# X-PLUG/Youku-mPLUG

Measured on NVIDIA H100. Metric: video-text samples/sec (pretrain 1.3B, 8f x 224^2), higher is better.
Workload: dtype bf16

## Files before the change

include/ymp.h:

```cpp
#ifndef YMP_H_
#define YMP_H_

#include <stddef.h>
#include <stdint.h>

#ifdef __cplusplus
extern "C" {
#endif

#define YMP_OK 0
#define YMP_EINVAL (-1)
#define YMP_ECUDA (-2)
#define YMP_ENOSUP (-3)

const char* ymp_last_error(void);
int ymp_abi_version(void);
uint64_t ymp_launch_count(void);
int ymp_set_pdl(int on);

typedef struct ymp_dropout_spec {
  const uint64_t* rng;
  uint32_t site;
  float p;
} ymp_dropout_spec;
#define YMP_DROP_SITE_EMBED 0u
#define YMP_DROP_SITE_ATTN(layer) (4u * (layer) + 1u)
#define YMP_DROP_SITE_BDA_ATTN(layer) (4u * (layer) + 2u)
#define YMP_DROP_SITE_BDA_MLP(layer) (4u * (layer) + 3u)

#define YMP_ACT_NONE 0
#define YMP_ACT_GELU_ERF 1
#define YMP_ACT_GELU_TANH 2

#define YMP_DT_BF16 0
#define YMP_DT_F32 1

typedef struct ymp_gemm_args {
  const void* A;
  const void* B;
  void* D;
  int32_t M, N, K;
  int32_t lda, ldb, ldd;
  int32_t a_mn_major, b_mn_major;
  const void* bias;
  const void* residual;
  int32_t ldr;
  int32_t act;
  void* aux_out;
  const void* aux_in;
  int32_t out_dtype;
  int32_t accumulate;
  int32_t split_k;
  float alpha;
  int32_t tile_n;
  int32_t res_row_mod;
  int32_t d_row_block;
  int32_t d_row_stride;
  int32_t residual_dtype;
  ymp_dropout_spec drop;
  int32_t im2col_P, im2col_B, im2col_C, im2col_T, im2col_H, im2col_W;
} ymp_gemm_args;

int ymp_gemm(const ymp_gemm_args* a, void* stream);

typedef struct ymp_gemm_skinny_args {
  const void* x;
  const void* w;
  const void* bias;
  const void* residual;
  void* y;
  int32_t M, N, K, ldx, ldw, ldr, ldy;
  int32_t act, residual_dtype, out_dtype;
  void* y2;
  const int64_t* y2_off_dev;
  int64_t ldy2, y2_off_stride;
  const void* ln_gamma;
  const void* ln_beta;
  void* ln_out;
  uint32_t* ln_counter;
  int32_t ld_ln;
  float ln_eps;
} ymp_gemm_skinny_args;
int ymp_gemm_skinny(const ymp_gemm_skinny_args* a, void* stream);
int ymp_gemm_skinny_wide(const ymp_gemm_skinny_args* a, void* stream);

typedef struct ymp_layernorm_args {
  const void* x;
  const void* gamma;
  const void* beta;
  void* y;
  float* mean;
  float* rstd;
  const int32_t* in_rows;
  int32_t rows, D, ldx, ldy;
  float eps;
  int32_t x_dtype;
  int32_t y_dtype;
} ymp_layernorm_args;
int ymp_layernorm_fwd(const ymp_layernorm_args* a, void* stream);

typedef struct ymp_layernorm_bwd_args {
  const void* dy;
  const void* x;
  const void* gamma;
  const float* mean;
  const float* rstd;
  const void* add;
  void* dx;
  float* dgamma;
  float* dbeta;
  const int32_t* in_rows;
  int32_t rows, D, ldx, lddy, ldadd;
  int32_t x_dtype;
  void* dx_drop;
  ymp_dropout_spec drop;
} ymp_layernorm_bwd_args;
// ... 140 lines not shown
```

youku-mplug_b200/csrc/gemm_wgmma.cu:

```cuda
#include <cuda.h>

#include "common.h"
#include "philox.cuh"
#include "ptx.cuh"
#include "wgmma.cuh"

namespace ymp {

constexpr int BM = 128;
constexpr int BK = 64;
constexpr int WGMMA_K = 16;
constexpr int GEMM_THREADS = 3 * 128;
constexpr int A_STAGE_BYTES = BM * BK * 2;

struct GemmKParams {
  void* D;
  const __nv_bfloat16* bias;
  const void* residual;
  __nv_bfloat16* aux_out;
  const __nv_bfloat16* aux_in;
  int M, N, K;
  int ldd, ldr;
  int a_mn, b_mn;
  int act, out_f32, accumulate, split_k;
  int kb_per_split;
  int res_row_mod;
  int d_row_block, d_row_stride;
  int res_f32;
  int n_fast;
  float alpha;
  int im2col_T, im2col_N, im2col_Wp;
  DropSpec drop;
  int has_drop;
};

template <int BN>
struct GemmCfg {
  static constexpr int NSTAGE = (BN == 256) ? 4 : 6;
  static constexpr int B_STAGE_BYTES = BN * BK * 2;
  static constexpr int STAGE_BYTES = A_STAGE_BYTES + B_STAGE_BYTES;
  static constexpr int STG_LD = BN + 4;
  static_assert(BM * STG_LD * 4 <= NSTAGE * STAGE_BYTES, "epilogue staging reuses the operand ring");
  static constexpr int SMEM_BYTES = NSTAGE * STAGE_BYTES + 256 + 1024;
};

template <int BN>
struct EpiCfg {
  static constexpr int TPR = BN / 8;
  static constexpr int RPP = 256 / TPR;
  static constexpr int GROUP = 4;
  static_assert(BM % (RPP * GROUP) == 0, "row groups tile BM");
};

__device__ __forceinline__ uint2 ld_bf16x4(const __nv_bfloat16* p) { return __ldg(reinterpret_cast<const uint2*>(p)); }
__device__ __forceinline__ void st_bf16x4(__nv_bfloat16* p, const float* f) {
  *reinterpret_cast<uint2*>(p) = make_uint2(pack_bf16(f[0], f[1]), pack_bf16(f[2], f[3]));
}

constexpr int EPI_ANY = -1;
enum { EPI_AUX_NONE = 0, EPI_AUX_MUL = 1, EPI_AUX_GELU_ERF = 2, EPI_AUX_GELU_TANH = 3 };
enum { EPI_OUT_BF16 = 0, EPI_OUT_F32 = 1, EPI_OUT_ATOMIC = 2 };
constexpr int epi_kind(int aux, int res_f32, int out) { return aux * 16 + res_f32 * 4 + out; }
template <int KIND>
struct EpiFlags {
  bool aux_in, aux_out, residual, res_f32, out_f32, accumulate;
  int act;
  __device__ __forceinline__ explicit EpiFlags(const GemmKParams& p) {
    if constexpr (KIND == EPI_ANY) {
      aux_in = p.aux_in != nullptr; aux_out = p.aux_out != nullptr; act = p.act;
      residual = p.residual != nullptr; res_f32 = p.res_f32 != 0;
      out_f32 = p.out_f32 != 0; accumulate = p.accumulate != 0;
    } else {
      constexpr int aux = KIND / 16, out = KIND % 4;
      aux_in = aux == EPI_AUX_MUL; aux_out = aux >= EPI_AUX_GELU_ERF;
      act = aux == EPI_AUX_GELU_ERF ? YMP_ACT_GELU_ERF : aux == EPI_AUX_GELU_TANH ? YMP_ACT_GELU_TANH : YMP_ACT_NONE;
      residual = res_f32 = (KIND / 4) % 4 != 0;
      out_f32 = out != EPI_OUT_BF16; accumulate = out == EPI_OUT_ATOMIC;
    }
  }
};
__device__ __forceinline__ int epi_kind_of(const GemmKParams& p) {
  const int aux = p.aux_in ? EPI_AUX_MUL
                  : (p.act == YMP_ACT_NONE && !p.aux_out) ? EPI_AUX_NONE
                  : (p.act == YMP_ACT_GELU_ERF && p.aux_out) ? EPI_AUX_GELU_ERF
                  : (p.act == YMP_ACT_GELU_TANH && p.aux_out) ? EPI_AUX_GELU_TANH : -1;
  if (aux < 0 || p.has_drop || (p.residual && !p.res_f32)) return EPI_ANY;
  return epi_kind(aux, p.residual ? 1 : 0, !p.out_f32 ? EPI_OUT_BF16 : p.accumulate ? EPI_OUT_ATOMIC : EPI_OUT_F32);
}

struct EpiIn {
  uint32_t res[8];
  uint32_t aux[4];
};
template <int KIND>
__device__ __forceinline__ void epilogue_fetch(const GemmKParams& p, int row, const int (&col)[2], bool full, EpiIn& in) {
  const EpiFlags<KIND> f(p);
  if (row >= p.M || !full) return;
  if (f.aux_in) {
#pragma unroll
    for (int q = 0; q < 2; ++q) {
      const uint2 a = ld_bf16x4(p.aux_in + (size_t)row * p.ldd + col[q]);
      in.aux[2 * q] = a.x; in.aux[2 * q + 1] = a.y;
// ... 76 lines not shown
        for (int i = 0; i < 8; ++i) v[i] += __uint_as_float(in.res[i]);
      } else {
#pragma unroll
        for (int i = 0; i < 4; ++i) { v[2 * i] += bf16_lo(in.res[i]); v[2 * i + 1] += bf16_hi(in.res[i]); }
      }
    }
#pragma unroll
    for (int q = 0; q < 2; ++q) {
      if (!f.out_f32) {
        st_bf16x4(reinterpret_cast<__nv_bfloat16*>(p.D) + doff[q], v + 4 * q);
      } else if (!f.accumulate) {
        *reinterpret_cast<float4*>(reinterpret_cast<float*>(p.D) + doff[q]) = make_float4(v[4 * q], v[4 * q + 1], v[4 * q + 2], v[4 * q + 3]);
      } else {
        asm volatile("red.global.add.v4.f32 [%0], {%1, %2, %3, %4};" ::"l"(reinterpret_cast<float*>(p.D) + doff[q]),
                     "f"(v[4 * q]), "f"(v[4 * q + 1]), "f"(v[4 * q + 2]), "f"(v[4 * q + 3])
                     : "memory");
      }
    }
  } else {
#pragma unroll
    for (int i = 0; i < 8; ++i) {
      const int c = col[i >> 2] + (i & 3);
      if (c < p.N) {
        float x = v[i];
        if (p.bias) x += __bfloat162float(p.bias[c]);
        const size_t off = (size_t)row * p.ldd + c, doff = (size_t)drow * p.ldd + c;
        if (f.aux_in) {
          x *= __bfloat162float(p.aux_in[off]);
        } else if (f.act == YMP_ACT_GELU_ERF) {
          float d; x = gelu_erf_both(x, d);
          if (f.aux_out) p.aux_out[off] = __float2bfloat16(d);
        } else if (f.act == YMP_ACT_GELU_TANH) {
          float d; x = gelu_tanh_both(x, d);
          if (f.aux_out) p.aux_out[off] = __float2bfloat16(d);
        } else if (f.aux_out) {
          p.aux_out[off] = __float2bfloat16(x);
        }
        if constexpr (DROP) {
          const uint4 w = drop_words(ds, (uint32_t)row, (uint32_t)c >> 2);
          const uint32_t wc = (c & 3) == 0 ? w.x : (c & 3) == 1 ? w.y : (c & 3) == 2 ? w.z : w.w;
          x = wc >= ds.thresh ? x * ds.scale : 0.f;
        }
        if (f.residual)
          x += f.res_f32 ? reinterpret_cast<const float*>(p.residual)[(size_t)rrow * p.ldr + c]
                         : __bfloat162float(reinterpret_cast<const __nv_bfloat16*>(p.residual)[(size_t)rrow * p.ldr + c]);
        if (!f.out_f32) reinterpret_cast<__nv_bfloat16*>(p.D)[doff] = __float2bfloat16(x);
        else if (!f.accumulate) reinterpret_cast<float*>(p.D)[doff] = x;
        else atomicAdd(reinterpret_cast<float*>(p.D) + doff, x);
      }
    }
  }
}

constexpr int IM2COL_SUB_BYTES = BM * 32;
__device__ __forceinline__ void load_a_im2col(uint8_t* sa, const CUtensorMap* tma, uint64_t* bar, int m0, int kb,
                                              const GemmKParams& p) {
  const int T = p.im2col_T, c = kb >> 2, y0 = (kb & 3) * 4;
  const int pt = m0 / T;
  for (int i = 0; i < BM / T; ++i) {
    const int g = pt + i, b = g / p.im2col_N, n = g - b * p.im2col_N;
    const int ny = n / p.im2col_Wp, nx = n - ny * p.im2col_Wp;
#pragma unroll
    for (int ks = 0; ks < 4; ++ks) {
      uint8_t* dst = sa + ks * IM2COL_SUB_BYTES + i * T * 32;
      tma_load_5d(dst, tma, bar, nx * 16, ny * 16 + y0 + ks, 0, c, b);
    }
  }
}
__device__ __forceinline__ void named_sync(int id, int n) { asm volatile("bar.sync %0, %1;" ::"r"(id), "r"(n) : "memory"); }

template <int BN, int KIND>
__device__ __forceinline__ void epilogue_rows(const GemmKParams& p, const float* stg, int m_blk, int n_blk) {
  using Cfg = GemmCfg<BN>;
  using Epi = EpiCfg<BN>;
  DropState ds;
  if (KIND == EPI_ANY && p.has_drop) ds = drop_state(p.drop);
  const int et = threadIdx.x - 128, tj = et % Epi::TPR, tr = et / Epi::TPR;
  const int col[2] = {n_blk * BN + 4 * tj, n_blk * BN + BN / 2 + 4 * tj};
  const bool full = col[1] + 4 <= p.N;
  uint32_t bias[4];
  if (p.bias && full) {
#pragma unroll
    for (int q = 0; q < 2; ++q) {
      const uint2 b = ld_bf16x4(p.bias + col[q]);
      bias[2 * q] = b.x; bias[2 * q + 1] = b.y;
    }
  }
#pragma unroll 1
  for (int lr0 = tr; lr0 < BM; lr0 += Epi::RPP * Epi::GROUP) {
    EpiIn in[Epi::GROUP];
#pragma unroll
    for (int u = 0; u < Epi::GROUP; ++u) epilogue_fetch<KIND>(p, m_blk * BM + lr0 + u * Epi::RPP, col, full, in[u]);
#pragma unroll
    for (int u = 0; u < Epi::GROUP; ++u) {
      const int lr = lr0 + u * Epi::RPP;
      const float4 a = *reinterpret_cast<const float4*>(stg + lr * Cfg::STG_LD + 4 * tj);
      const float4 b = *reinterpret_cast<const float4*>(stg + lr * Cfg::STG_LD + BN / 2 + 4 * tj);
      float v[8] = {a.x, a.y, a.z, a.w, b.x, b.y, b.z, b.w};
      if (KIND == EPI_ANY && p.has_drop) epilogue_row<true, KIND>(p, v, m_blk * BM + lr, col, full, bias, in[u], ds);
      else epilogue_row<false, KIND>(p, v, m_blk * BM + lr, col, full, bias, in[u], ds);
    }
  }
}

template <int BN, int AMN, int BMN>
__global__ void __launch_bounds__(GEMM_THREADS, 1)
gemm_bf16_wgmma_kernel(const __grid_constant__ CUtensorMap tma_a, const __grid_constant__ CUtensorMap tma_b,
                       const GemmKParams p) {
  using Cfg = GemmCfg<BN>;
  constexpr int NSTAGE = Cfg::NSTAGE;
  extern __shared__ uint8_t smem_raw[];
  const uint32_t raw_addr = smem_u32(smem_raw);
  uint8_t* smem = smem_raw + ((1024u - (raw_addr & 1023u)) & 1023u);
  uint8_t* smem_a = smem;
  uint8_t* smem_b = smem + NSTAGE * A_STAGE_BYTES;
  uint64_t* full_bar = reinterpret_cast<uint64_t*>(smem + NSTAGE * Cfg::STAGE_BYTES);
  uint64_t* empty_bar = full_bar + NSTAGE;

  const int wg = threadIdx.x >> 7;
  const int num_m = (p.M + BM - 1) / BM;
  const int num_n = (p.N + BN - 1) / BN;
  const int kb_total = (p.K + BK - 1) / BK;
  const int ks = blockIdx.x % p.split_k;
  const int t = blockIdx.x / p.split_k;
  const int m_blk = p.n_fast ? t / num_n : t % num_m;
  const int n_blk = p.n_fast ? t % num_n : t / num_m;
  const int kb0 = ks * p.kb_per_split;
  const int kb1 = min(kb_total, kb0 + p.kb_per_split);

  if (threadIdx.x == 0) {
    tma_prefetch_desc(&tma_a);
    tma_prefetch_desc(&tma_b);
    for (int i = 0; i < NSTAGE; ++i) {
      mbar_init(&full_bar[i], 1);
      mbar_init(&empty_bar[i], 2);
    }
    fence_mbar_init();
  }
  __syncthreads();

  if (wg == 0) {
    if (threadIdx.x == 0) {
      int stage = 0;
      uint32_t phase = 0;
      for (int kb = kb0; kb < kb1; ++kb) {
        mbar_wait(&empty_bar[stage], phase ^ 1);
        mbar_expect_tx(&full_bar[stage], Cfg::STAGE_BYTES);
        uint8_t* sa = smem_a + stage * A_STAGE_BYTES;
        uint8_t* sb = smem_b + stage * Cfg::B_STAGE_BYTES;
        if (p.im2col_T) {
          load_a_im2col(sa, &tma_a, &full_bar[stage], m_blk * BM, kb, p);
        } else if (!AMN) {
          tma_load_2d(sa, &tma_a, &full_bar[stage], kb * BK, m_blk * BM);
        } else {
#pragma unroll
          for (int c = 0; c < BM / 64; ++c)
            tma_load_2d(sa + c * (64 * BK * 2), &tma_a, &full_bar[stage], m_blk * BM + c * 64, kb * BK);
        }
        if (!BMN) {
          tma_load_2d(sb, &tma_b, &full_bar[stage], kb * BK, n_blk * BN);
        } else {
#pragma unroll
          for (int c = 0; c < BN / 64; ++c)
            tma_load_2d(sb + c * (64 * BK * 2), &tma_b, &full_bar[stage], n_blk * BN + c * 64, kb * BK);
        }
        if (++stage == NSTAGE) { stage = 0; phase ^= 1; }
      }
    }
    return;
  }

  const int cw = wg - 1;
  float acc[BN / 2];
#pragma unroll
  for (int i = 0; i < BN / 2; ++i) acc[i] = 0.f;
  {
    int stage = 0;
    uint32_t phase = 0;
    int prev = -1;
    wgmma_fence_acc(acc);
    for (int kb = kb0; kb < kb1; ++kb) {
      mbar_wait(&full_bar[stage], phase);
      const uint32_t sa = smem_u32(smem_a + stage * A_STAGE_BYTES);
      const uint32_t sb = smem_u32(smem_b + stage * Cfg::B_STAGE_BYTES);
      wgmma_fence();
#pragma unroll
      for (int k = 0; k < BK / WGMMA_K; ++k) {
        const uint64_t da = p.im2col_T ? make_smem_desc(sa + k * IM2COL_SUB_BYTES + cw * 64 * 32, 16, 256, 3)
                            : AMN ? make_smem_desc(sa + cw * 8192 + k * WGMMA_K * 128, 64 * BK * 2, 1024, 1)
                                  : make_smem_desc(sa + cw * 8192 + k * WGMMA_K * 2, 16, 1024, 1);
        const uint64_t db = BMN ? make_smem_desc(sb + k * WGMMA_K * 128, 64 * BK * 2, 1024, 1)
                                : make_smem_desc(sb + k * WGMMA_K * 2, 16, 1024, 1);
        if constexpr (BN == 256) wgmma_m64n256<AMN, BMN>(acc, da, db, 1u);
        else wgmma_m64n128<AMN, BMN>(acc, da, db, 1u);
      }
      wgmma_commit();
      wgmma_wait<1>();
      if (prev >= 0 && (threadIdx.x & 127) == 0) mbar_arrive(&empty_bar[prev]);
      prev = stage;
      if (++stage == NSTAGE) { stage = 0; phase ^= 1; }
    }
    wgmma_wait<0>();
    wgmma_fence_acc(acc);
  }

  named_sync(1, 256);
  float* stg = reinterpret_cast<float*>(smem);
  {
    const int lt = threadIdx.x & 127, r0 = cw * 64 + (lt >> 5) * 16 + ((lt & 31) >> 2), c0 = 2 * (lt & 3);
#pragma unroll
    for (int j = 0; j < BN / 8; ++j) {
      *reinterpret_cast<float2*>(stg + r0 * Cfg::STG_LD + 8 * j + c0) = make_float2(acc[4 * j], acc[4 * j + 1]);
      *reinterpret_cast<float2*>(stg + (r0 + 8) * Cfg::STG_LD + 8 * j + c0) = make_float2(acc[4 * j + 2], acc[4 * j + 3]);
    }
  }
  named_sync(1, 256);
  switch (epi_kind_of(p)) {
#define YMP_EPI_CASE(aux, res, out) \
    case epi_kind(aux, res, out): epilogue_rows<BN, epi_kind(aux, res, out)>(p, stg, m_blk, n_blk); break;
    YMP_EPI_CASE(EPI_AUX_NONE, 0, EPI_OUT_BF16)
    YMP_EPI_CASE(EPI_AUX_NONE, 1, EPI_OUT_F32)
    YMP_EPI_CASE(EPI_AUX_NONE, 0, EPI_OUT_ATOMIC)
    YMP_EPI_CASE(EPI_AUX_GELU_ERF, 0, EPI_OUT_BF16)
    YMP_EPI_CASE(EPI_AUX_GELU_TANH, 0, EPI_OUT_BF16)
    YMP_EPI_CASE(EPI_AUX_MUL, 0, EPI_OUT_BF16)
#undef YMP_EPI_CASE
    default: epilogue_rows<BN, EPI_ANY>(p, stg, m_blk, n_blk);
  }
}

typedef CUresult (*EncodeTiledFn)(CUtensorMap*, CUtensorMapDataType, cuuint32_t, void*,
                                  const cuuint64_t*, const cuuint64_t*, const cuuint32_t*,
                                  const cuuint32_t*, CUtensorMapInterleave, CUtensorMapSwizzle,
                                  CUtensorMapL2promotion, CUtensorMapFloatOOBfill);

static EncodeTiledFn get_encode_fn() {
  static EncodeTiledFn fn = nullptr;
  static bool tried = false;
  if (!tried) {
    tried = true;
    void* f = nullptr;
    cudaDriverEntryPointQueryResult q;
    if (cudaGetDriverEntryPoint("cuTensorMapEncodeTiled", &f, cudaEnableDefault, &q) == cudaSuccess &&
        q == cudaDriverEntryPointSuccess)
      fn = reinterpret_cast<EncodeTiledFn>(f);
    else
      cudaGetLastError();
  }
  return fn;
}

static int make_map(CUtensorMap* m, const void* ptr, uint64_t inner, uint64_t outer, uint64_t ld,
                    uint32_t box_inner, uint32_t box_outer) {
  EncodeTiledFn fn = get_encode_fn();
  if (!fn) return set_error(YMP_ECUDA, "cuTensorMapEncodeTiled entry point unavailable (no driver?)");
  cuuint64_t dims[2] = {inner, outer};
  cuuint64_t strides[1] = {ld * 2};
  cuuint32_t box[2] = {box_inner, box_outer};
  cuuint32_t estr[2] = {1, 1};
  CUresult r = fn(m, CU_TENSOR_MAP_DATA_TYPE_BFLOAT16, 2, const_cast<void*>(ptr), dims, strides, box,
                  estr, CU_TENSOR_MAP_INTERLEAVE_NONE, CU_TENSOR_MAP_SWIZZLE_128B,
                  CU_TENSOR_MAP_L2_PROMOTION_L2_256B, CU_TENSOR_MAP_FLOAT_OOB_FILL_NONE);
  if (r != CUDA_SUCCESS)
    return set_error(YMP_ECUDA, "cuTensorMapEncodeTiled failed (%d): inner=%llu outer=%llu ld=%llu",
                     (int)r, (unsigned long long)inner, (unsigned long long)outer,
                     (unsigned long long)ld);
  return YMP_OK;
}

static int make_video_map(CUtensorMap* m, const ymp_gemm_args* a) {
  EncodeTiledFn fn = get_encode_fn();
  if (!fn) return set_error(YMP_ECUDA, "cuTensorMapEncodeTiled entry point unavailable (no driver?)");
  const cuuint64_t W = a->im2col_W, H = a->im2col_H, T = a->im2col_T, C = a->im2col_C, B = a->im2col_B;
  cuuint64_t dims[5] = {W, H, T, C, B};
  cuuint64_t strides[4] = {W * 2, H * W * 2, T * H * W * 2, C * T * H * W * 2};
  cuuint32_t box[5] = {16, 1, (cuuint32_t)T, 1, 1};
  cuuint32_t estr[5] = {1, 1, 1, 1, 1};
  CUresult r = fn(m, CU_TENSOR_MAP_DATA_TYPE_BFLOAT16, 5, const_cast<void*>(a->A), dims, strides, box, estr,
                  CU_TENSOR_MAP_INTERLEAVE_NONE, CU_TENSOR_MAP_SWIZZLE_32B, CU_TENSOR_MAP_L2_PROMOTION_L2_256B,
                  CU_TENSOR_MAP_FLOAT_OOB_FILL_NONE);
  if (r != CUDA_SUCCESS) return set_error(YMP_ECUDA, "cuTensorMapEncodeTiled (video, 5-D) failed (%d)", (int)r);
  return YMP_OK;
}

template <int BN, int AMN, int BMN>
static int launch_gemm_t(const CUtensorMap& ta, const CUtensorMap& tb, const GemmKParams& kp, int grid, cudaStream_t stream) {
  using Cfg = GemmCfg<BN>;
  static DeviceOnce once;
  if (once.first())
    YMP_CUDA(cudaFuncSetAttribute(gemm_bf16_wgmma_kernel<BN, AMN, BMN>, cudaFuncAttributeMaxDynamicSharedMemorySize,
                                  Cfg::SMEM_BYTES));
  gemm_bf16_wgmma_kernel<BN, AMN, BMN><<<grid, GEMM_THREADS, Cfg::SMEM_BYTES, stream>>>(ta, tb, kp);
  YMP_LAUNCH_CHECK();
  return YMP_OK;
}

template <int BN>
static int launch_gemm(const ymp_gemm_args* a, const GemmKParams& kp, cudaStream_t stream) {
  CUtensorMap ta, tb;
  int rc;
  if (a->im2col_P) rc = make_video_map(&ta, a);
  else if (!a->a_mn_major) rc = make_map(&ta, a->A, a->K, a->M, a->lda, BK, BM);
  else rc = make_map(&ta, a->A, a->M, a->K, a->lda, 64, BK);
  if (rc) return rc;
  if (!a->b_mn_major) rc = make_map(&tb, a->B, a->K, a->N, a->ldb, BK, BN);
  else rc = make_map(&tb, a->B, a->N, a->K, a->ldb, 64, BK);
  if (rc) return rc;
  const int num_m = (a->M + BM - 1) / BM, num_n = (a->N + BN - 1) / BN;
  const int grid = num_m * num_n * kp.split_k;
  switch (kp.a_mn * 2 + kp.b_mn) {
    case 0: return launch_gemm_t<BN, 0, 0>(ta, tb, kp, grid, stream);
    case 1: return launch_gemm_t<BN, 0, 1>(ta, tb, kp, grid, stream);
    case 2: return launch_gemm_t<BN, 1, 0>(ta, tb, kp, grid, stream);
    default: return launch_gemm_t<BN, 1, 1>(ta, tb, kp, grid, stream);
  }
}

}

extern "C" int ymp_gemm(const ymp_gemm_args* a, void* stream) {
  using namespace ymp;
  YMP_CHECK_ARG(a != nullptr, "ymp_gemm: null args");
  YMP_CHECK_ARG(a->A && a->B && a->D, "ymp_gemm: null A/B/D");
  YMP_CHECK_ARG(a->M > 0 && a->N > 0 && a->K > 0, "ymp_gemm: bad shape M=%d N=%d K=%d", a->M, a->N, a->K);
  if (a->im2col_P) {
    const int P = a->im2col_P, T = a->im2col_T;
    YMP_CHECK_ARG(P == 16 && T > 0 && T % 8 == 0 && 128 % T == 0 && a->im2col_H % P == 0 && a->im2col_W % P == 0 && !a->a_mn_major,
                  "ymp_gemm(im2col): needs P = 16, T %% 8 == 0, 128 %% T == 0, H, W multiples of P (P=%d T=%d H=%d W=%d)", P, T,
                  a->im2col_H, a->im2col_W);
    const long rows = (long)a->im2col_B * (a->im2col_H / P) * (a->im2col_W / P) * T;
    YMP_CHECK_ARG(a->M == rows && a->K == a->im2col_C * P * P, "ymp_gemm(im2col): needs M = B*N*T, K = C*P*P (M=%d K=%d)", a->M, a->K);
  }
  const bool ia = a->im2col_P != 0;
  YMP_CHECK_ARG((ia || a->lda % 8 == 0) && a->ldb % 8 == 0, "ymp_gemm: lda/ldb must be multiples of 8 (lda=%d ldb=%d)", a->lda, a->ldb);
  YMP_CHECK_ARG(aligned16(a->A) && aligned16(a->B) && aligned16(a->D), "ymp_gemm: A/B/D must be 16-byte aligned");
  YMP_CHECK_ARG(ia || a->lda >= (a->a_mn_major ? a->M : a->K), "ymp_gemm: lda too small");
  YMP_CHECK_ARG(a->ldb >= (a->b_mn_major ? a->N : a->K), "ymp_gemm: ldb too small");
  YMP_CHECK_ARG(a->ldd >= a->N && a->ldd % 8 == 0, "ymp_gemm: ldd must be >= N and a multiple of 8 (ldd=%d)", a->ldd);
  YMP_CHECK_ARG(a->act >= 0 && a->act <= 2, "ymp_gemm: bad act %d", a->act);
  YMP_CHECK_ARG(!a->residual || (a->ldr >= a->N && a->ldr % 8 == 0 && aligned16(a->residual)), "ymp_gemm: bad residual ld/alignment");
  YMP_CHECK_ARG(a->residual_dtype == YMP_DT_BF16 || a->residual_dtype == YMP_DT_F32, "ymp_gemm: bad residual_dtype");
  YMP_CHECK_ARG(!a->bias || aligned16(a->bias), "ymp_gemm: bias must be 16-byte aligned");
  YMP_CHECK_ARG(!a->aux_out || aligned16(a->aux_out), "ymp_gemm: aux_out alignment");
  YMP_CHECK_ARG(!a->aux_in || aligned16(a->aux_in), "ymp_gemm: aux_in alignment");
  YMP_CHECK_ARG(!(a->accumulate && a->out_dtype != YMP_DT_F32), "ymp_gemm: accumulate needs fp32 output");
  YMP_CHECK_ARG(!(a->accumulate && (a->bias || a->aux_out || a->aux_in || a->act || a->residual)),
                "ymp_gemm: accumulate mode supports only alpha and bias-free linear epilogue");
  YMP_CHECK_ARG(a->res_row_mod >= 0 && a->d_row_block >= 0 && (a->d_row_block == 0 || a->d_row_stride >= a->d_row_block),
                "ymp_gemm: bad res_row_mod / d_row_block / d_row_stride");
  YMP_CHECK_ARG(!(a->drop.rng && a->drop.p > 0.f) || (a->drop.p < 1.f && !a->aux_out && !a->accumulate),
                "ymp_gemm: dropout needs 0 < p < 1 and is not combined with aux_out / accumulate");
  YMP_CHECK_ARG(a->tile_n == 0 || a->tile_n == 128 || a->tile_n == 256 || a->tile_n == 512,
                "ymp_gemm: tile_n must be 0 (auto), 128, 256 or 512 (the widest tile: 256 columns on sm_90)");

  const int kb_total = (a->K + BK - 1) / BK;
  const int sms = num_sms();
  int bn = a->tile_n == 512 ? 256 : a->tile_n;
  if (a->im2col_P && bn == 0) bn = (a->N <= 128) ? 128 : 256;
  if (bn == 0) {
    const long t256 = (long)((a->M + BM - 1) / BM) * ((a->N + 255) / 256);
    bn = (a->N <= 128 || (t256 < sms && a->split_k <= 1 && !a->accumulate)) ? 128 : 256;
  }
  int split = a->split_k;
  if (split <= 0) {
    split = 1;
    if (a->accumulate) {
      const long tiles = (long)((a->M + BM - 1) / BM) * ((a->N + bn - 1) / bn);
      const long workers = sms;
      long best = -1;
      for (int sp = 1; sp <= 64 && sp * 8 <= kb_total; ++sp) {
        const long waves = (tiles * sp + workers - 1) / workers;
        const long cost = waves * ((kb_total + sp - 1) / sp + 24);
        if (best < 0 || cost < best) { best = cost; split = sp; }
      }
    }
  }
  YMP_CHECK_ARG(split == 1 || (a->accumulate && a->out_dtype == YMP_DT_F32), "ymp_gemm: split_k>1 needs accumulate=1 and fp32 output");
  if (split > kb_total) split = kb_total;
  int per = (kb_total + split - 1) / split;
  split = (kb_total + per - 1) / per;

  GemmKParams kp;
  kp.D = a->D;
  kp.bias = reinterpret_cast<const __nv_bfloat16*>(a->bias);
  kp.residual = a->residual;
  kp.res_f32 = (a->residual_dtype == YMP_DT_F32) ? 1 : 0;
  kp.aux_out = reinterpret_cast<__nv_bfloat16*>(a->aux_out);
  kp.aux_in = reinterpret_cast<const __nv_bfloat16*>(a->aux_in);
  kp.M = a->M; kp.N = a->N; kp.K = a->K;
  kp.ldd = a->ldd; kp.ldr = a->ldr;
  kp.a_mn = a->a_mn_major ? 1 : 0; kp.b_mn = a->b_mn_major ? 1 : 0;
  kp.act = a->act; kp.out_f32 = (a->out_dtype == YMP_DT_F32); kp.accumulate = a->accumulate ? 1 : 0;
  kp.split_k = split; kp.kb_per_split = per;
  kp.alpha = a->alpha;
  kp.n_fast = ((long)a->M >= (long)a->N) ? 1 : 0;
  kp.res_row_mod = a->res_row_mod; kp.d_row_block = a->d_row_block; kp.d_row_stride = a->d_row_stride;
  kp.im2col_T = a->im2col_P ? a->im2col_T : 0;
  kp.im2col_Wp = a->im2col_P ? a->im2col_W / a->im2col_P : 0;
  kp.im2col_N = a->im2col_P ? (a->im2col_H / a->im2col_P) * kp.im2col_Wp : 0;
  kp.has_drop = (a->drop.rng && a->drop.p > 0.f) ? 1 : 0;
  kp.drop.rng = a->drop.rng; kp.drop.site = a->drop.site; kp.drop.p = a->drop.p;
  cudaStream_t st = reinterpret_cast<cudaStream_t>(stream);
  if (bn == 256) return launch_gemm<256>(a, kp, st);
  return launch_gemm<128>(a, kp, st);
}
```

youku-mplug_b200/ymp/lib.py:

```python
import ctypes as C
import os

_HERE = os.path.dirname(os.path.abspath(__file__))
LIB_PATH = os.path.join(_HERE, "libymp_b200.so")


class YmpError(RuntimeError):
    pass


if not os.path.exists(LIB_PATH):
    raise ImportError(
        f"{LIB_PATH} not found: build it with `make -C youku-mplug_b200/csrc` "
        "(or `python -c 'import __graft_entry__ as g; g.build()'`). There is no CPU fallback."
    )

lib = C.CDLL(LIB_PATH)

ACT_NONE, ACT_GELU_ERF, ACT_GELU_TANH = 0, 1, 2
MASK_NONE, MASK_CAUSAL, MASK_BLOCK = 0, 1, 2
DT_BF16, DT_F32 = 0, 1

c_i32 = C.c_int32
c_vp = C.c_void_p
# ... 83 lines not shown
    _fields_ = [("video", c_vp), ("out", c_vp), ("B", c_i32), ("C", c_i32), ("T", c_i32), ("H", c_i32),
                ("W", c_i32), ("P", c_i32), ("ldo", c_i32)]


class ClipArgs(C.Structure):
    _fields_ = [("frames", c_vp), ("out", c_vp), ("lut", c_vp), ("B", c_i32), ("T", c_i32), ("H", c_i32), ("W", c_i32),
                ("C", c_i32)]


class EmbedArgs(C.Structure):
    _fields_ = [("ids", c_vp), ("table", c_vp), ("pos", c_vp), ("out", c_vp), ("B", c_i32), ("L", c_i32),
                ("S", c_i32), ("row_offset", c_i32), ("hidden", c_i32), ("vocab", c_i32), ("ldo", c_i32),
                ("out_dtype", c_i32)]


class CeArgs(C.Structure):
    _fields_ = [("logits", c_vp), ("labels", c_vp), ("loss", c_vp), ("lse", c_vp), ("grad_rows", c_vp),
                ("dlogits", c_vp), ("rows", c_i32), ("V", c_i32), ("ld", c_i32)]


class ColsumArgs(C.Structure):
    _fields_ = [("in_", c_vp), ("out", c_vp), ("R", c_i32), ("C", c_i32), ("ld", c_i32)]


class GroupArgs(C.Structure):
    _fields_ = [("in_", c_vp), ("out", c_vp), ("G", c_i32), ("T", c_i32), ("C", c_i32), ("ld_in", c_i32),
                ("ld_out", c_i32), ("broadcast", c_i32), ("scale", C.c_float)]


class AdamwArgs(C.Structure):
    _fields_ = [("master", c_vp), ("param", c_vp), ("grad", c_vp), ("m", c_vp), ("v", c_vp), ("sumsq", c_vp),
                ("n", C.c_int64), ("step", c_i32), ("lr", C.c_float), ("beta1", C.c_float), ("beta2", C.c_float),
                ("eps", C.c_float), ("weight_decay", C.c_float), ("grad_scale", C.c_float),
                ("max_grad_norm", C.c_float), ("hyper", c_vp), ("zero_grad", c_i32)]


lib.ymp_last_error.restype = C.c_char_p
lib.ymp_abi_version.restype = C.c_int
lib.ymp_launch_count.restype = C.c_uint64
lib.ymp_attn_last_path.restype = C.c_int
lib.ymp_set_pdl.restype = C.c_int
lib.ymp_set_pdl.argtypes = [C.c_int]
ATTN_PATH_MMA_SYNC, ATTN_PATH_WGMMA, ATTN_PATH_SMALL, ATTN_PATH_DECODE = 0, 1, 2, 3


def _declare(name, argstruct):
    fn = getattr(lib, name)
    fn.restype = C.c_int
    fn.argtypes = [C.POINTER(argstruct), c_vp]
    return fn


_gemm = _declare("ymp_gemm", GemmArgs)
_gemm_skinny = _declare("ymp_gemm_skinny", GemmSkinnyArgs)
_gemm_skinny_wide = _declare("ymp_gemm_skinny_wide", GemmSkinnyArgs)
_ln_fwd = _declare("ymp_layernorm_fwd", LayerNormArgs)
_ln_bwd = _declare("ymp_layernorm_bwd", LayerNormBwdArgs)
_attn_fwd = _declare("ymp_attn_fwd", AttnArgs)
_attn_bwd = _declare("ymp_attn_bwd", AttnBwdArgs)
_im2col = _declare("ymp_im2col", Im2colArgs)
_clip = _declare("ymp_clip_normalize", ClipArgs)
_embed = _declare("ymp_embed_gather", EmbedArgs)
_ce_fwd = _declare("ymp_ce_fwd", CeArgs)
_ce_bwd = _declare("ymp_ce_bwd", CeArgs)
_colsum = _declare("ymp_colsum", ColsumArgs)
_group = _declare("ymp_group_reduce", GroupArgs)
_adamw = _declare("ymp_adamw", AdamwArgs)
_dropout = _declare("ymp_dropout", DropoutArgs)
_sumsq = lib.ymp_sumsq
_sumsq.restype = C.c_int
_sumsq.argtypes = [c_vp, C.c_int64, c_vp, c_vp]


def check(rc, what):
    if rc != 0:
        raise YmpError(f"{what} failed ({rc}): {lib.ymp_last_error().decode()}")


def launch_count():
    return int(lib.ymp_launch_count())


def set_pdl(on):
    return int(lib.ymp_set_pdl(int(bool(on))))


def attn_last_path():
    return int(lib.ymp_attn_last_path())


def ptr(t):
    return None if t is None else t.data_ptr()


def cur_stream():
    import torch
    return torch.cuda.current_stream().cuda_stream


def call(fn, args, what):
    check(fn(C.byref(args), cur_stream()), what)
```

youku-mplug_b200/ymp/ops.py:

```python
import torch

from . import lib as L
from .lib import (ACT_NONE, ACT_GELU_ERF, ACT_GELU_TANH, DT_BF16, DT_F32,
                  MASK_NONE, MASK_CAUSAL, MASK_BLOCK)

bf16 = torch.bfloat16


class Drop:
    __slots__ = ("rng", "site", "p")

    def __init__(self, rng, site, p):
        assert rng.dtype == torch.int64 and rng.numel() == 2 and rng.is_cuda
        self.rng, self.site, self.p = rng, int(site), float(p)


def _set_drop(spec, drop):
    if drop is not None and drop.p > 0.0:
        spec.rng, spec.site, spec.p = drop.rng.data_ptr(), drop.site, drop.p


def site_embed():
    return 0


def site_attn(layer):
    return 4 * layer + 1


def site_bda_attn(layer):
    return 4 * layer + 2


def site_bda_mlp(layer):
    return 4 * layer + 3


def dropout(x, drop, out=None, row0=0):
    _chk2d(x, "x")
    out = x if out is None else out
    assert out.dtype == x.dtype and out.shape == x.shape and x.dtype in (bf16, torch.float32)
    a = L.DropoutArgs()
    a.x, a.y, a.rows, a.cols, a.ldx, a.ldy = x.data_ptr(), out.data_ptr(), x.shape[0], x.shape[1], x.stride(0), out.stride(0)
    a.dtype, a.row0 = (DT_F32 if x.dtype == torch.float32 else DT_BF16), row0
    _set_drop(a.drop, drop)
    L.call(L._dropout, a, "ymp_dropout")
    return out


def _chk2d(t, name):
    assert t.is_cuda and t.dim() == 2 and t.stride(1) == 1, f"{name}: need 2-D row-major CUDA tensor"


def gemm(a, b, *, a_t=False, b_t=False, bias=None, residual=None, act=ACT_NONE, aux_out=None,
         aux_in=None, out=None, out_dtype=bf16, accumulate=False, split_k=0, alpha=1.0, tile_n=0,
         res_row_mod=0, d_row_block=0, d_row_stride=0, drop=None, _im2col=None):
    _chk2d(a, "a"); _chk2d(b, "b")
    assert a.dtype == bf16 and b.dtype == bf16
    if _im2col is not None:
        P, vB, vC, vT, vH, vW = _im2col
        M, K = vB * (vH // P) * (vW // P) * vT, vC * P * P
    else:
        M, K = (a.shape[1], a.shape[0]) if a_t else (a.shape[0], a.shape[1])
    N, Kb = (b.shape[1], b.shape[0]) if b_t else (b.shape[0], b.shape[1])
    assert K == Kb, f"gemm: K mismatch {K} vs {Kb}"
    if out is None:
        out = torch.empty((M, N), device=a.device, dtype=out_dtype)
        assert not accumulate, "accumulate needs an explicit (zeroed or running) output"
    _chk2d(out, "out")
    if d_row_block:
        assert out.shape[1] == N and M % d_row_block == 0
        assert out.shape[0] >= (M // d_row_block - 1) * d_row_stride + d_row_block
    else:
        assert out.shape == (M, N), f"gemm: out shape {tuple(out.shape)} != {(M, N)}"
    g = L.GemmArgs()
    g.A, g.B, g.D = a.data_ptr(), b.data_ptr(), out.data_ptr()
    g.M, g.N, g.K = M, N, K
    g.lda, g.ldb, g.ldd = a.stride(0), b.stride(0), out.stride(0)
    g.a_mn_major, g.b_mn_major = int(a_t), int(b_t)
    g.bias = L.ptr(bias)
    g.residual = L.ptr(residual)
    g.ldr = residual.stride(0) if residual is not None else 0
    if residual is not None:
        assert residual.dtype in (bf16, torch.float32) and residual.stride(1) == 1
        g.residual_dtype = DT_F32 if residual.dtype == torch.float32 else DT_BF16
    g.act = act
    if aux_out is not None:
        assert aux_out.dtype == bf16 and aux_out.shape == (M, N) and aux_out.stride(0) == out.stride(0)
    if aux_in is not None:
        assert aux_in.dtype == bf16 and aux_in.shape == (M, N) and aux_in.stride(0) == out.stride(0)
    g.aux_out, g.aux_in = L.ptr(aux_out), L.ptr(aux_in)
    g.out_dtype = DT_F32 if out.dtype == torch.float32 else DT_BF16
    g.accumulate = int(accumulate)
    g.split_k = split_k
    g.alpha = alpha
    g.tile_n = tile_n
    g.res_row_mod, g.d_row_block, g.d_row_stride = res_row_mod, d_row_block, d_row_stride
    _set_drop(g.drop, drop)
    if _im2col is not None:
        g.im2col_P, g.im2col_B, g.im2col_C, g.im2col_T, g.im2col_H, g.im2col_W = _im2col
    L.call(L._gemm, g, "ymp_gemm")
    return out


SKINNY_MAX_ROWS = 8
SKINNY_WIDE_MAX_ROWS = 64


def gemm_skinny(x, w, *, bias=None, residual=None, act=ACT_NONE, out=None, out_dtype=bf16, out2=None, out2_row_stride=0,
                out2_off=None, ln=None):
    return _gemm_skinny(x, w, bias, residual, act, out, out_dtype, out2, out2_row_stride, out2_off, ln, wide=False)


def gemm_skinny_wide(x, w, *, bias=None, residual=None, act=ACT_NONE, out=None, out_dtype=bf16, out2=None, out2_row_stride=0,
                     out2_off=None, ln=None):
    return _gemm_skinny(x, w, bias, residual, act, out, out_dtype, out2, out2_row_stride, out2_off, ln, wide=True)


def _gemm_skinny(x, w, bias, residual, act, out, out_dtype, out2, out2_row_stride, out2_off, ln, wide):
    _chk2d(x, "x"); _chk2d(w, "w")
    assert x.dtype == bf16 and w.dtype == bf16 and x.shape[1] == w.shape[1] and (wide or x.shape[0] <= SKINNY_MAX_ROWS)
    M, K, N = x.shape[0], x.shape[1], w.shape[0]
    if out is None:
        out = torch.empty((M, N), device=x.device, dtype=out_dtype)
    _chk2d(out, "out")
    assert out.shape == (M, N)
    a = L.GemmSkinnyArgs()
    a.x, a.w, a.bias, a.residual, a.y = x.data_ptr(), w.data_ptr(), L.ptr(bias), L.ptr(residual), out.data_ptr()
    a.M, a.N, a.K, a.ldx, a.ldw, a.ldy = M, N, K, x.stride(0), w.stride(0), out.stride(0)
    if residual is not None:
        assert residual.dtype in (bf16, torch.float32) and residual.stride(1) == 1 and residual.shape == (M, N)
        a.ldr = residual.stride(0)
        a.residual_dtype = DT_F32 if residual.dtype == torch.float32 else DT_BF16
    a.act = act
    a.out_dtype = DT_F32 if out.dtype == torch.float32 else DT_BF16
    if out2 is not None:
        _chk2d(out2, "out2")
        assert out2.dtype == bf16 and out2.shape[1] == N and out2_off.dtype == torch.int64 and out2_off.numel() == 1
        assert out2.shape[0] >= (M - 1) * out2_row_stride + 1
        a.y2, a.y2_off_dev = out2.data_ptr(), out2_off.data_ptr()
        a.ldy2, a.y2_off_stride = out2_row_stride * out2.stride(0), out2.stride(0)
    ln_out = None
    if ln is not None:
        gamma, beta, eps, counter = ln
        assert out.dtype == torch.float32 and gamma.dtype == bf16 and beta.dtype == bf16 and counter.numel() == 1
        assert counter.dtype in (torch.int32, torch.uint32) and gamma.numel() == N and beta.numel() == N
        ln_out = torch.empty((M, N), device=x.device, dtype=bf16)
        a.ln_gamma, a.ln_beta, a.ln_out, a.ln_counter = gamma.data_ptr(), beta.data_ptr(), ln_out.data_ptr(), counter.data_ptr()
        a.ld_ln, a.ln_eps = ln_out.stride(0), eps
    if wide:
        L.call(L._gemm_skinny_wide, a, "ymp_gemm_skinny_wide")
    else:
        L.call(L._gemm_skinny, a, "ymp_gemm_skinny")
    return out if ln is None else (out, ln_out)
# ... 268 lines not shown
```

Baseline: 162.7.

## Add 192-row GEMM tile with producer-in-consumer pipeline and cost-model tile selection

```diff
diff --git a/include/ymp.h b/include/ymp.h
--- a/include/ymp.h
+++ b/include/ymp.h
@@ -62,6 +62,7 @@
 } ymp_gemm_args;
 
 int ymp_gemm(const ymp_gemm_args* a, void* stream);
+int ymp_gemm_tiled(const ymp_gemm_args* a, int tile_m, void* stream);
 
 typedef struct ymp_gemm_skinny_args {
   const void* x;
diff --git a/youku-mplug_b200/csrc/gemm_wgmma.cu b/youku-mplug_b200/csrc/gemm_wgmma.cu
--- a/youku-mplug_b200/csrc/gemm_wgmma.cu
+++ b/youku-mplug_b200/csrc/gemm_wgmma.cu
@@ -1,4 +1,6 @@
 #include <cuda.h>
+
+#include <algorithm>
 
 #include "common.h"
 #include "philox.cuh"
@@ -7,11 +9,9 @@
 
 namespace ymp {
 
-constexpr int BM = 128;
 constexpr int BK = 64;
 constexpr int WGMMA_K = 16;
-constexpr int GEMM_THREADS = 3 * 128;
-constexpr int A_STAGE_BYTES = BM * BK * 2;
+constexpr int SMEM_OPTIN_MAX = 232448;
 
 struct GemmKParams {
   void* D;
@@ -34,20 +34,28 @@
   int has_drop;
 };
 
-template <int BN>
+template <int BM, int BN>
 struct GemmCfg {
+  static_assert((BM == 128 && (BN == 128 || BN == 256)) || (BM == 192 && BN == 256), "tile shapes");
+  static constexpr int CONSUMERS = BM / 64;
+  static constexpr bool PRODUCER_WG = CONSUMERS == 2;
+  static constexpr int THREADS = 128 * (CONSUMERS + PRODUCER_WG);
+  static constexpr int FIRST_CONSUMER = THREADS - 128 * CONSUMERS;
   static constexpr int NSTAGE = (BN == 256) ? 4 : 6;
+  static constexpr int A_STAGE_BYTES = BM * BK * 2;
   static constexpr int B_STAGE_BYTES = BN * BK * 2;
   static constexpr int STAGE_BYTES = A_STAGE_BYTES + B_STAGE_BYTES;
   static constexpr int STG_LD = BN + 4;
   static_assert(BM * STG_LD * 4 <= NSTAGE * STAGE_BYTES, "epilogue staging reuses the operand ring");
   static constexpr int SMEM_BYTES = NSTAGE * STAGE_BYTES + 256 + 1024;
+  static_assert(SMEM_BYTES <= SMEM_OPTIN_MAX, "ring, barriers and alignment pad fit the opt-in shared memory");
 };
 
-template <int BN>
+template <int BM, int BN>
 struct EpiCfg {
+  static constexpr int THREADS = 2 * BM;
   static constexpr int TPR = BN / 8;
-  static constexpr int RPP = 256 / TPR;
+  static constexpr int RPP = THREADS / TPR;
   static constexpr int GROUP = 4;
   static_assert(BM % (RPP * GROUP) == 0, "row groups tile BM");
 };
@@ -230,12 +238,13 @@
   }
 }
 
-constexpr int IM2COL_SUB_BYTES = BM * 32;
+constexpr int IM2COL_BM = 128;
+constexpr int IM2COL_SUB_BYTES = IM2COL_BM * 32;
 __device__ __forceinline__ void load_a_im2col(uint8_t* sa, const CUtensorMap* tma, uint64_t* bar, int m0, int kb,
                                               const GemmKParams& p) {
   const int T = p.im2col_T, c = kb >> 2, y0 = (kb & 3) * 4;
   const int pt = m0 / T;
-  for (int i = 0; i < BM / T; ++i) {
+  for (int i = 0; i < IM2COL_BM / T; ++i) {
     const int g = pt + i, b = g / p.im2col_N, n = g - b * p.im2col_N;
     const int ny = n / p.im2col_Wp, nx = n - ny * p.im2col_Wp;
 #pragma unroll
@@ -247,13 +256,13 @@
 }
 __device__ __forceinline__ void named_sync(int id, int n) { asm volatile("bar.sync %0, %1;" ::"r"(id), "r"(n) : "memory"); }
 
-template <int BN, int KIND>
+template <int BM, int BN, int KIND>
 __device__ __forceinline__ void epilogue_rows(const GemmKParams& p, const float* stg, int m_blk, int n_blk) {
-  using Cfg = GemmCfg<BN>;
-  using Epi = EpiCfg<BN>;
+  using Cfg = GemmCfg<BM, BN>;
+  using Epi = EpiCfg<BM, BN>;
   DropState ds;
   if (KIND == EPI_ANY && p.has_drop) ds = drop_state(p.drop);
-  const int et = threadIdx.x - 128, tj = et % Epi::TPR, tr = et / Epi::TPR;
+  const int et = threadIdx.x - Cfg::FIRST_CONSUMER, tj = et % Epi::TPR, tr = et / Epi::TPR;
   const int col[2] = {n_blk * BN + 4 * tj, n_blk * BN + BN / 2 + 4 * tj};
   const bool full = col[1] + 4 <= p.N;
   uint32_t bias[4];
@@ -281,12 +290,14 @@
   }
 }
 
-template <int BN, int AMN, int BMN>
-__global__ void __launch_bounds__(GEMM_THREADS, 1)
+template <int BM, int BN, int AMN, int BMN>
+__global__ void __launch_bounds__(GemmCfg<BM, BN>::THREADS, 1)
 gemm_bf16_wgmma_kernel(const __grid_constant__ CUtensorMap tma_a, const __grid_constant__ CUtensorMap tma_b,
                        const GemmKParams p) {
-  using Cfg = GemmCfg<BN>;
+  using Cfg = GemmCfg<BM, BN>;
   constexpr int NSTAGE = Cfg::NSTAGE;
+  constexpr int A_STAGE_BYTES = Cfg::A_STAGE_BYTES;
+  constexpr bool IM2COL = BM == IM2COL_BM;
   extern __shared__ uint8_t smem_raw[];
   const uint32_t raw_addr = smem_u32(smem_raw);
   uint8_t* smem = smem_raw + ((1024u - (raw_addr & 1023u)) & 1023u);
@@ -311,44 +322,52 @@
     tma_prefetch_desc(&tma_b);
     for (int i = 0; i < NSTAGE; ++i) {
       mbar_init(&full_bar[i], 1);
-      mbar_init(&empty_bar[i], 2);
+      mbar_init(&empty_bar[i], Cfg::CONSUMERS);
     }
     fence_mbar_init();
   }
   __syncthreads();
 
-  if (wg == 0) {
-    if (threadIdx.x == 0) {
-      int stage = 0;
-      uint32_t phase = 0;
-      for (int kb = kb0; kb < kb1; ++kb) {
-        mbar_wait(&empty_bar[stage], phase ^ 1);
-        mbar_expect_tx(&full_bar[stage], Cfg::STAGE_BYTES);
-        uint8_t* sa = smem_a + stage * A_STAGE_BYTES;
-        uint8_t* sb = smem_b + stage * Cfg::B_STAGE_BYTES;
-        if (p.im2col_T) {
-          load_a_im2col(sa, &tma_a, &full_bar[stage], m_blk * BM, kb, p);
-        } else if (!AMN) {
-          tma_load_2d(sa, &tma_a, &full_bar[stage], kb * BK, m_blk * BM);
-        } else {
-#pragma unroll
-          for (int c = 0; c < BM / 64; ++c)
-            tma_load_2d(sa + c * (64 * BK * 2), &tma_a, &full_bar[stage], m_blk * BM + c * 64, kb * BK);
+  auto load_stage = [&](int kb, int stage) {
+    mbar_expect_tx(&full_bar[stage], Cfg::STAGE_BYTES);
+    uint8_t* sa = smem_a + stage * A_STAGE_BYTES;
+    uint8_t* sb = smem_b + stage * Cfg::B_STAGE_BYTES;
+    if (IM2COL && p.im2col_T) {
+      load_a_im2col(sa, &tma_a, &full_bar[stage], m_blk * BM, kb, p);
+    } else if (!AMN) {
+      tma_load_2d(sa, &tma_a, &full_bar[stage], kb * BK, m_blk * BM);
+    } else {
+#pragma unroll
+      for (int c = 0; c < BM / 64; ++c)
+        tma_load_2d(sa + c * (64 * BK * 2), &tma_a, &full_bar[stage], m_blk * BM + c * 64, kb * BK);
+    }
+    if (!BMN) {
+      tma_load_2d(sb, &tma_b, &full_bar[stage], kb * BK, n_blk * BN);
+    } else {
+#pragma unroll
+      for (int c = 0; c < BN / 64; ++c)
+        tma_load_2d(sb + c * (64 * BK * 2), &tma_b, &full_bar[stage], n_blk * BN + c * 64, kb * BK);
+    }
+  };
+
+  if constexpr (Cfg::PRODUCER_WG) {
+    if (wg == 0) {
+      if (threadIdx.x == 0) {
+        int stage = 0;
+        uint32_t phase = 0;
+        for (int kb = kb0; kb < kb1; ++kb) {
+          mbar_wait(&empty_bar[stage], phase ^ 1);
+          load_stage(kb, stage);
+          if (++stage == NSTAGE) { stage = 0; phase ^= 1; }
         }
-        if (!BMN) {
-          tma_load_2d(sb, &tma_b, &full_bar[stage], kb * BK, n_blk * BN);
-        } else {
-#pragma unroll
-          for (int c = 0; c < BN / 64; ++c)
-            tma_load_2d(sb + c * (64 * BK * 2), &tma_b, &full_bar[stage], n_blk * BN + c * 64, kb * BK);
-        }
-        if (++stage == NSTAGE) { stage = 0; phase ^= 1; }
-      }
-    }
-    return;
-  }
-
-  const int cw = wg - 1;
+      }
+      return;
+    }
+  } else if (threadIdx.x == 0) {
+    for (int i = 0; i < NSTAGE && kb0 + i < kb1; ++i) load_stage(kb0 + i, i);
+  }
+
+  const int cw = wg - Cfg::PRODUCER_WG;
   float acc[BN / 2];
 #pragma unroll
   for (int i = 0; i < BN / 2; ++i) acc[i] = 0.f;
@@ -364,7 +383,7 @@
       wgmma_fence();
 #pragma unroll
       for (int k = 0; k < BK / WGMMA_K; ++k) {
-        const uint64_t da = p.im2col_T ? make_smem_desc(sa + k * IM2COL_SUB_BYTES + cw * 64 * 32, 16, 256, 3)
+        const uint64_t da = IM2COL && p.im2col_T ? make_smem_desc(sa + k * IM2COL_SUB_BYTES + cw * 64 * 32, 16, 256, 3)
                             : AMN ? make_smem_desc(sa + cw * 8192 + k * WGMMA_K * 128, 64 * BK * 2, 1024, 1)
                                   : make_smem_desc(sa + cw * 8192 + k * WGMMA_K * 2, 16, 1024, 1);
         const uint64_t db = BMN ? make_smem_desc(sb + k * WGMMA_K * 128, 64 * BK * 2, 1024, 1)
@@ -375,6 +394,12 @@
       wgmma_commit();
       wgmma_wait<1>();
       if (prev >= 0 && (threadIdx.x & 127) == 0) mbar_arrive(&empty_bar[prev]);
+      if constexpr (!Cfg::PRODUCER_WG) {
+        if (threadIdx.x == 0 && prev >= 0 && kb - 1 + NSTAGE < kb1) {
+          mbar_wait(&empty_bar[prev], ((kb - 1 - kb0) / NSTAGE) & 1);
+          load_stage(kb - 1 + NSTAGE, prev);
+        }
+      }
       prev = stage;
       if (++stage == NSTAGE) { stage = 0; phase ^= 1; }
     }
@@ -382,7 +407,7 @@
     wgmma_fence_acc(acc);
   }
 
-  named_sync(1, 256);
+  named_sync(1, 128 * Cfg::CONSUMERS);
   float* stg = reinterpret_cast<float*>(smem);
   {
     const int lt = threadIdx.x & 127, r0 = cw * 64 + (lt >> 5) * 16 + ((lt & 31) >> 2), c0 = 2 * (lt & 3);
@@ -392,10 +417,10 @@
       *reinterpret_cast<float2*>(stg + (r0 + 8) * Cfg::STG_LD + 8 * j + c0) = make_float2(acc[4 * j + 2], acc[4 * j + 3]);
     }
   }
-  named_sync(1, 256);
+  named_sync(1, 128 * Cfg::CONSUMERS);
   switch (epi_kind_of(p)) {
 #define YMP_EPI_CASE(aux, res, out) \
-    case epi_kind(aux, res, out): epilogue_rows<BN, epi_kind(aux, res, out)>(p, stg, m_blk, n_blk); break;
+    case epi_kind(aux, res, out): epilogue_rows<BM, BN, epi_kind(aux, res, out)>(p, stg, m_blk, n_blk); break;
     YMP_EPI_CASE(EPI_AUX_NONE, 0, EPI_OUT_BF16)
     YMP_EPI_CASE(EPI_AUX_NONE, 1, EPI_OUT_F32)
     YMP_EPI_CASE(EPI_AUX_NONE, 0, EPI_OUT_ATOMIC)
@@ -403,7 +428,7 @@
     YMP_EPI_CASE(EPI_AUX_GELU_TANH, 0, EPI_OUT_BF16)
     YMP_EPI_CASE(EPI_AUX_MUL, 0, EPI_OUT_BF16)
 #undef YMP_EPI_CASE
-    default: epilogue_rows<BN, EPI_ANY>(p, stg, m_blk, n_blk);
+    default: epilogue_rows<BM, BN, EPI_ANY>(p, stg, m_blk, n_blk);
   }
 }
 
@@ -461,19 +486,19 @@
   return YMP_OK;
 }
 
-template <int BN, int AMN, int BMN>
+template <int BM, int BN, int AMN, int BMN>
 static int launch_gemm_t(const CUtensorMap& ta, const CUtensorMap& tb, const GemmKParams& kp, int grid, cudaStream_t stream) {
-  using Cfg = GemmCfg<BN>;
+  using Cfg = GemmCfg<BM, BN>;
   static DeviceOnce once;
   if (once.first())
-    YMP_CUDA(cudaFuncSetAttribute(gemm_bf16_wgmma_kernel<BN, AMN, BMN>, cudaFuncAttributeMaxDynamicSharedMemorySize,
+    YMP_CUDA(cudaFuncSetAttribute(gemm_bf16_wgmma_kernel<BM, BN, AMN, BMN>, cudaFuncAttributeMaxDynamicSharedMemorySize,
                                   Cfg::SMEM_BYTES));
-  gemm_bf16_wgmma_kernel<BN, AMN, BMN><<<grid, GEMM_THREADS, Cfg::SMEM_BYTES, stream>>>(ta, tb, kp);
+  gemm_bf16_wgmma_kernel<BM, BN, AMN, BMN><<<grid, Cfg::THREADS, Cfg::SMEM_BYTES, stream>>>(ta, tb, kp);
   YMP_LAUNCH_CHECK();
   return YMP_OK;
 }
 
-template <int BN>
+template <int BM, int BN>
 static int launch_gemm(const ymp_gemm_args* a, const GemmKParams& kp, cudaStream_t stream) {
   CUtensorMap ta, tb;
   int rc;
@@ -487,16 +512,39 @@
   const int num_m = (a->M + BM - 1) / BM, num_n = (a->N + BN - 1) / BN;
   const int grid = num_m * num_n * kp.split_k;
   switch (kp.a_mn * 2 + kp.b_mn) {
-    case 0: return launch_gemm_t<BN, 0, 0>(ta, tb, kp, grid, stream);
-    case 1: return launch_gemm_t<BN, 0, 1>(ta, tb, kp, grid, stream);
-    case 2: return launch_gemm_t<BN, 1, 0>(ta, tb, kp, grid, stream);
-    default: return launch_gemm_t<BN, 1, 1>(ta, tb, kp, grid, stream);
-  }
-}
-
-}
-
-extern "C" int ymp_gemm(const ymp_gemm_args* a, void* stream) {
+    case 0: return launch_gemm_t<BM, BN, 0, 0>(ta, tb, kp, grid, stream);
+    case 1: return launch_gemm_t<BM, BN, 0, 1>(ta, tb, kp, grid, stream);
+    case 2: return launch_gemm_t<BM, BN, 1, 0>(ta, tb, kp, grid, stream);
+    default: return launch_gemm_t<BM, BN, 1, 1>(ta, tb, kp, grid, stream);
+  }
+}
+
+struct TileCost { double t, f, f_acc; };
+constexpr TileCost TILE_COST_128 = {0.78, 5.0, 14.7};
+constexpr TileCost TILE_COST_192 = {1.09, 8.0, 20.0};
+
+struct GemmPlan { int split; double us; };
+static GemmPlan plan_gemm(long tiles, int kb_total, int split, bool accumulate, int sms, const TileCost& c) {
+  auto cost = [&](int sp) {
+    const long waves = (tiles * sp + sms - 1) / sms;
+    return waves * (((kb_total + sp - 1) / sp) * c.t + (accumulate ? c.f_acc : c.f));
+  };
+  if (split > 0) return {split, cost(std::min(split, kb_total))};
+  GemmPlan best{1, cost(1)};
+  if (accumulate) {
+    for (int sp = 2; sp <= 64 && sp * 8 <= kb_total; ++sp) {
+      const double us = cost(sp);
+      if (us < best.us) best = {sp, us};
+    }
+  }
+  return best;
+}
+
+}
+
+extern "C" int ymp_gemm(const ymp_gemm_args* a, void* stream) { return ymp_gemm_tiled(a, 0, stream); }
+
+extern "C" int ymp_gemm_tiled(const ymp_gemm_args* a, int tile_m, void* stream) {
   using namespace ymp;
   YMP_CHECK_ARG(a != nullptr, "ymp_gemm: null args");
   YMP_CHECK_ARG(a->A && a->B && a->D, "ymp_gemm: null A/B/D");
@@ -530,29 +578,28 @@
                 "ymp_gemm: dropout needs 0 < p < 1 and is not combined with aux_out / accumulate");
   YMP_CHECK_ARG(a->tile_n == 0 || a->tile_n == 128 || a->tile_n == 256 || a->tile_n == 512,
                 "ymp_gemm: tile_n must be 0 (auto), 128, 256 or 512 (the widest tile: 256 columns on sm_90)");
+  YMP_CHECK_ARG(tile_m == 0 || tile_m == 128 || tile_m == 192, "ymp_gemm: tile_m must be 0 (auto), 128 or 192 (tile_m=%d)", tile_m);
+  YMP_CHECK_ARG(tile_m != 192 || (a->tile_n != 128 && !a->im2col_P),
+                "ymp_gemm: tile_m = 192 needs the 256-column tile and no fused im2col operand");
 
   const int kb_total = (a->K + BK - 1) / BK;
   const int sms = num_sms();
   int bn = a->tile_n == 512 ? 256 : a->tile_n;
+  if (tile_m == 192) bn = 256;
   if (a->im2col_P && bn == 0) bn = (a->N <= 128) ? 128 : 256;
   if (bn == 0) {
-    const long t256 = (long)((a->M + BM - 1) / BM) * ((a->N + 255) / 256);
+    const long t256 = (long)((a->M + 127) / 128) * ((a->N + 255) / 256);
     bn = (a->N <= 128 || (t256 < sms && a->split_k <= 1 && !a->accumulate)) ? 128 : 256;
   }
-  int split = a->split_k;
-  if (split <= 0) {
-    split = 1;
-    if (a->accumulate) {
-      const long tiles = (long)((a->M + BM - 1) / BM) * ((a->N + bn - 1) / bn);
-      const long workers = sms;
-      long best = -1;
-      for (int sp = 1; sp <= 64 && sp * 8 <= kb_total; ++sp) {
-        const long waves = (tiles * sp + workers - 1) / workers;
-        const long cost = waves * ((kb_total + sp - 1) / sp + 24);
-        if (best < 0 || cost < best) { best = cost; split = sp; }
-      }
-    }
-  }
+  const bool acc = a->accumulate != 0;
+  const long tiles128 = (long)((a->M + 127) / 128) * ((a->N + bn - 1) / bn);
+  GemmPlan plan = plan_gemm(tiles128, kb_total, a->split_k, acc, sms, TILE_COST_128);
+  int bm = 128;
+  if (tile_m == 192 || (tile_m == 0 && bn == 256 && !a->im2col_P)) {
+    const GemmPlan p192 = plan_gemm((long)((a->M + 191) / 192) * ((a->N + 255) / 256), kb_total, a->split_k, acc, sms, TILE_COST_192);
+    if (tile_m == 192 || p192.us < plan.us) { plan = p192; bm = 192; }
+  }
+  int split = plan.split;
   YMP_CHECK_ARG(split == 1 || (a->accumulate && a->out_dtype == YMP_DT_F32), "ymp_gemm: split_k>1 needs accumulate=1 and fp32 output");
   if (split > kb_total) split = kb_total;
   int per = (kb_total + split - 1) / split;
@@ -579,6 +626,7 @@
   kp.has_drop = (a->drop.rng && a->drop.p > 0.f) ? 1 : 0;
   kp.drop.rng = a->drop.rng; kp.drop.site = a->drop.site; kp.drop.p = a->drop.p;
   cudaStream_t st = reinterpret_cast<cudaStream_t>(stream);
-  if (bn == 256) return launch_gemm<256>(a, kp, st);
-  return launch_gemm<128>(a, kp, st);
-}
+  if (bm == 192) return launch_gemm<192, 256>(a, kp, st);
+  if (bn == 256) return launch_gemm<128, 256>(a, kp, st);
+  return launch_gemm<128, 128>(a, kp, st);
+}
diff --git a/youku-mplug_b200/ymp/lib.py b/youku-mplug_b200/ymp/lib.py
--- a/youku-mplug_b200/ymp/lib.py
+++ b/youku-mplug_b200/ymp/lib.py
@@ -159,6 +159,9 @@
 
 
 _gemm = _declare("ymp_gemm", GemmArgs)
+_gemm_tiled = lib.ymp_gemm_tiled
+_gemm_tiled.restype = C.c_int
+_gemm_tiled.argtypes = [C.POINTER(GemmArgs), C.c_int, c_vp]
 _gemm_skinny = _declare("ymp_gemm_skinny", GemmSkinnyArgs)
 _gemm_skinny_wide = _declare("ymp_gemm_skinny_wide", GemmSkinnyArgs)
 _ln_fwd = _declare("ymp_layernorm_fwd", LayerNormArgs)
diff --git a/youku-mplug_b200/ymp/ops.py b/youku-mplug_b200/ymp/ops.py
--- a/youku-mplug_b200/ymp/ops.py
+++ b/youku-mplug_b200/ymp/ops.py
@@ -54,7 +54,7 @@
 
 def gemm(a, b, *, a_t=False, b_t=False, bias=None, residual=None, act=ACT_NONE, aux_out=None,
          aux_in=None, out=None, out_dtype=bf16, accumulate=False, split_k=0, alpha=1.0, tile_n=0,
-         res_row_mod=0, d_row_block=0, d_row_stride=0, drop=None, _im2col=None):
+         tile_m=0, res_row_mod=0, d_row_block=0, d_row_stride=0, drop=None, _im2col=None):
     _chk2d(a, "a"); _chk2d(b, "b")
     assert a.dtype == bf16 and b.dtype == bf16
     if _im2col is not None:
@@ -99,7 +99,7 @@
     _set_drop(g.drop, drop)
     if _im2col is not None:
         g.im2col_P, g.im2col_B, g.im2col_C, g.im2col_T, g.im2col_H, g.im2col_W = _im2col
-    L.call(L._gemm, g, "ymp_gemm")
+    L.check(L._gemm_tiled(L.C.byref(g), tile_m, L.cur_stream()), "ymp_gemm")
     return out
 
 
```

Result: faster. 168.9, median of 6 (+3.8%).
